# OCR-D/ocrd_keraslm

Hardware: AMD Instinct MI355X
Metric: chars/sec training (stacked-LSTM forward+backward+Adam) (higher is better)
Workload: dtype bf16; 1 GPU; cfg2: depth=2 width=512 length=256 V=256 1 context, stateful training, 3072 streams/GPU, synthetic 10M-char corpus (SURVEY.md 8d); streams_per_gpu=3072, global_batch=3072, seq_len=256, parallelism=dp1

## Files before the change

include/keraslm_hip.h:

```cpp
#ifndef KERASLM_HIP_H
#define KERASLM_HIP_H

#include <stddef.h>
#include <stdint.h>

#ifdef __cplusplus
extern "C" {
#endif

#define KL_ABI_VERSION 1

enum {
  KL_OK = 0,
  KL_ERR_SHAPE = 1,
  KL_ERR_LAUNCH = 2,
  KL_ERR_STATE = 3,
  KL_ERR_WORKSPACE = 4,
  KL_ERR_ARG = 5
};

#define KL_PREC_BF16 1
#define KL_PREC_SPLIT 3

typedef struct kl_config {
// ... 47 lines not shown

int kl_assemble_windows(const int32_t* corpus, size_t n_corpus, const int64_t* plan, int B, int T, int n_ctx, int32_t* idx,
                        int32_t* ctx, int32_t* tgt, void* stream);

int kl_adam_step(kl_handle* h, const float* grads, float* m, float* v, int t, float lr, float b1, float b2,
                 float eps, float clip, void* stream);
int kl_adam_step_scaled(kl_handle* h, const float* grads, float grad_scale, float* m, float* v, int t, float lr,
                        float b1, float b2, float eps, float clip, void* stream);

size_t kl_step_workspace_bytes(const kl_handle* h, int n);
int kl_step_batch(kl_handle* h, int n, const int32_t* idx, const int32_t* ctx, float* pool, const int32_t* slot_in,
                  const int32_t* slot_out, float* probs, void* ws, size_t ws_bytes, void* stream);

void* kl_host_alloc(size_t bytes);
void kl_host_free(void* p);
size_t kl_step_host_workspace_bytes(const kl_handle* h, int n);
int kl_step_batch_host(kl_handle* h, int n, const int32_t* idx, const int32_t* ctx, const int32_t* slot_in,
                       const int32_t* slot_out, const int32_t* target, float* pool, int head_k, float* probs_host,
                       float* heads_host, uint32_t* done_host, uint32_t ticket, void* ws, size_t ws_bytes, void* stream);
size_t kl_walk_workspace_bytes(const kl_handle* h, int n, int total);
size_t kl_walk_stage_bytes(const kl_handle* h, int n, int total);
int kl_walk_batch_host(kl_handle* h, int n, const int32_t* len, const int32_t* idx, const int32_t* target,
                       const int32_t* ctx, const int32_t* slot_in, const int32_t* slot_step, float* pool, int head_k,
                       float* tprob_host, float* heads_host, void* stage_host, uint32_t* done_host, uint32_t ticket,
                       void* ws, size_t ws_bytes, void* stream);
int kl_step_wait(const uint32_t* done_host, uint32_t ticket, double timeout_s);

size_t kl_beam_workspace_bytes(const kl_handle* h, int rows, int fan);
int kl_beam_expand(kl_handle* h, int rows, int fan, float floor, const float* probs, const uint8_t* valid,
                   const float* cum_in, const int32_t* slot_new, int32_t zero_slot, int32_t* idx_next,
                   int32_t* slot_in_next, float* cum_next, int32_t* parent_log, int32_t* idx_log, float* cum_log,
                   int32_t* n_live, void* ws, size_t ws_bytes, void* stream);

size_t kl_sample_workspace_bytes(const kl_handle* h, int rows);
int kl_sample_pick(kl_handle* h, int rows, const float* probs, const uint8_t* valid, float temperature, int top_k,
                   float floor, uint64_t seed, uint32_t step, const float* cum_in, int32_t* idx_next, float* cum_next,
                   float* u_log, void* ws, size_t ws_bytes, void* stream);
int kl_sample_pick_from(kl_handle* h, int rows, uint32_t row0, const float* probs, const uint8_t* valid, float temperature,
                        int top_k, float floor, uint64_t seed, uint32_t step, const float* cum_in, int32_t* idx_next,
                        float* cum_next, float* u_log, void* ws, size_t ws_bytes, void* stream);

int kl_state_dist2(const kl_handle* h, int n, const float* pool, const int32_t* a, const int32_t* b, int k,
                   float* out, void* stream);

int kl_trace_enable(kl_handle* h, int on);
int kl_trace_read(kl_handle* h, int kind, int* n_launches, float* total_ms, int* persistent,
                  double* flops_per_launch);
const char* kl_trace_kernel_name(kl_handle* h, int kind);

int kl_test_gemm_tn(const uint16_t* A, const uint16_t* B, void* C, const float* bias, int M, int N, int K, long lda,
                    long ldb, long ldc, int out_mode, int splits, void* stream);
int kl_test_gemm_an(const uint16_t* A_km, const uint16_t* B, float* C, int M, int N, int K, long lda_km, long ldb,
                    long ldc, int c_transposed, int b_km, void* stream);
size_t kl_test_segment_sums_ws_bytes(int B, int T, int n_ctx, int V, int R);
int kl_test_segment_sums_share(int B, int T);
int kl_test_segment_sums(const uint16_t* dZ, long ld, int B, int T, int cols, const int32_t* idx, const int32_t* ctx, int n_ctx,
                         int V, int R, float* dEK, float* dCtxK, void* ws, void* stream);
int kl_test_thin_gemm(const float* A, long lda, const uint16_t* WT_hi, const uint16_t* WT_lo, long ldw, int M, int N,
                      int K, float* C, long ldc, int split, void* stream);
int kl_test_softmax_ce(float* logits, long ld, int rows, int V, const int32_t* tgt, int B, int T, float inv_count, uint16_t* dlogits,
                       long ld_dl, float* rowstat, float* loss_acc, int last_only, void* stream);
int kl_test_logits_ce_ws(const uint16_t* X, const uint16_t* E, const int32_t* tgt, uint16_t* dlogits, float* rowstat, int B, int T,
                         float inv_count, int last_only, void* stream);
int kl_test_logits_ce_w128(const uint16_t* X, const uint16_t* E, const uint16_t* ET, const int32_t* tgt, uint16_t* dlogits, float* dH,
                           float* rowstat, int B, int T, int V, int Vp, float inv_count, int last_only, void* stream);
int kl_test_dh_ws(const uint16_t* dlogits, const uint16_t* ET, uint16_t* dH, long M, void* stream);
int kl_test_rate_topk(const float* logits, long ld, int rows, int V, const int32_t* tgt, int B, int T, int K,
                      float* tprob, int32_t* alt_id, float* alt_p, int32_t* rank, void* stream);

typedef struct kl_window_view {
  int32_t depth, width, B, T;
  int32_t g_interleaved, c_in_cb, dh_bf16, p_bf16_mask, scan2_rows, reserved[7];
  uint64_t off_H[16], off_C[16], off_Cb[16], off_G[16], off_dZ[16];
} kl_window_view;
int kl_test_window_view(const kl_handle* h, int B, int T, const void* ws, kl_window_view* out);

#ifdef __cplusplus
}
#endif
#endif
```

ocrd_keraslm_amd/csrc/api.hip:

```cpp
#include <hip/hip_runtime.h>
#include <stdio.h>
#include <stdlib.h>
#include <string.h>
#include <time.h>

#include <functional>
#include <utility>

#include <vector>

#include "kl_common.h"
#include "kl_kernels.h"

namespace {

inline size_t align_up(size_t x, size_t a) { return (x + a - 1) / a * a; }
inline int round_up_i(int x, int a) { return (x + a - 1) / a * a; }

struct Carver {
  unsigned char* base;
  size_t off = 0;
  explicit Carver(void* b) : base(reinterpret_cast<unsigned char*>(b)) {}
  template <typename T>
  T* take(size_t count) {
// ... 2022 lines not shown
                   int32_t* parent_log, int32_t* idx_log, float* cum_log, int32_t* n_live, void* ws, size_t ws_bytes,
                   void* stream) {
  if (!h || !probs || !cum_in || !slot_new || !idx_next || !slot_in_next || !cum_next || !parent_log || !idx_log || !cum_log ||
      !n_live)
    return KL_ERR_ARG;
  if (rows < 1 || rows > KL_BEAM_MAX_ROWS || fan < 1 || fan > KL_BEAM_MAX_FAN) return KL_ERR_ARG;
  if (!ws || ws_bytes < kl_beam_ws_bytes(rows, fan)) return KL_ERR_WORKSPACE;
  KlBeamExpand a;
  memset(&a, 0, sizeof(a));
  a.rows = rows; a.fan = fan; a.V = h->cfg.voc_size; a.floor = floor;
  a.probs = probs; a.valid = valid; a.cum_in = cum_in; a.slot_new = slot_new; a.zero_slot = zero_slot;
  a.idx_next = idx_next; a.slot_in_next = slot_in_next; a.cum_next = cum_next;
  a.parent_log = parent_log; a.idx_log = idx_log; a.cum_log = cum_log; a.n_live = n_live;
  return kl_launch_beam_expand(a, ws, (hipStream_t)stream);
}

size_t kl_sample_workspace_bytes(const kl_handle* h, int rows) {
  if (!h || rows < 1 || rows > KL_SAMPLE_MAX_ROWS) return 0;
  return kl_sample_ws_bytes(rows, h->cfg.voc_size);
}

int kl_sample_pick_from(kl_handle* h, int rows, uint32_t row0, const float* probs, const uint8_t* valid, float temperature,
                        int top_k, float floor, uint64_t seed, uint32_t step, const float* cum_in, int32_t* idx_next,
                        float* cum_next, float* u_log, void* ws, size_t ws_bytes, void* stream) {
  if (!h || !probs || !cum_in || !idx_next || !cum_next) return KL_ERR_ARG;
  if (rows < 1 || rows > KL_SAMPLE_MAX_ROWS || top_k < 0 || top_k > KL_SAMPLE_MAX_TOPK) return KL_ERR_ARG;
  if (!(temperature >= 0.f) || temperature == INFINITY || !(floor >= 0.f)) return KL_ERR_ARG;
  if (!ws || ws_bytes < kl_sample_ws_bytes(rows, h->cfg.voc_size)) return KL_ERR_WORKSPACE;
  KlSamplePick a;
  memset(&a, 0, sizeof(a));
  a.rows = rows; a.V = h->cfg.voc_size; a.top_k = top_k; a.temperature = temperature; a.floor = floor;
  a.key0 = (unsigned)(seed & 0xffffffffu); a.key1 = (unsigned)(seed >> 32); a.step = step; a.row0 = row0;
  a.probs = probs; a.valid = valid; a.cum_in = cum_in; a.idx_next = idx_next; a.cum_next = cum_next; a.u_log = u_log;
  return kl_launch_sample_pick(a, ws, (hipStream_t)stream);
}

int kl_sample_pick(kl_handle* h, int rows, const float* probs, const uint8_t* valid, float temperature, int top_k, float floor,
                   uint64_t seed, uint32_t step, const float* cum_in, int32_t* idx_next, float* cum_next, float* u_log, void* ws,
                   size_t ws_bytes, void* stream) {
  return kl_sample_pick_from(h, rows, 0, probs, valid, temperature, top_k, floor, seed, step, cum_in, idx_next, cum_next, u_log,
                             ws, ws_bytes, stream);
}

int kl_test_gemm_tn(const uint16_t* A, const uint16_t* B, void* C, const float* bias, int M, int N, int K, long lda,
                    long ldb, long ldc, int out_mode, int splits, void* stream) {
  return kl_launch_gemm_tn(A, B, C, bias, M, N, K, lda, ldb, ldc, out_mode, splits, 1.f, (hipStream_t)stream);
}

int kl_test_gemm_an(const uint16_t* A_km, const uint16_t* B, float* C, int M, int N, int K, long lda_km, long ldb,
                    long ldc, int c_transposed, int b_km, void* stream) {
  return kl_launch_gemm_an(A_km, B, C, M, N, K, lda_km, ldb, ldc, c_transposed, (hipStream_t)stream, b_km);
}

size_t kl_test_segment_sums_ws_bytes(int B, int T, int n_ctx, int V, int R) {
  if (B < 1 || T < 1 || V < 1 || n_ctx < 0 || (n_ctx > 0 && R < 1)) return 0;
  return kl_segment_sums_ws_bytes(B, T, n_ctx, V, R);
}

int kl_test_segment_sums_share(int B, int T) { return B < 1 || T < 1 ? 0 : kl_segment_sums_share((long)B * T); }

int kl_test_segment_sums(const uint16_t* dZ, long ld, int B, int T, int cols, const int32_t* idx, const int32_t* ctx, int n_ctx,
                         int V, int R, float* dEK, float* dCtxK, void* ws, void* stream) {
  return kl_launch_segment_sums(dZ, ld, B, T, cols, idx, ctx, n_ctx, V, R, dEK, dCtxK, ws, (hipStream_t)stream);
}

int kl_test_thin_gemm(const float* A, long lda, const uint16_t* WT_hi, const uint16_t* WT_lo, long ldw, int M, int N,
                      int K, float* C, long ldc, int split, void* stream) {
  KlOperand op;
  memset(&op, 0, sizeof(op));
  op.A = A; op.lda = lda; op.a_is_f32 = 1; op.WT_hi = WT_hi; op.WT_lo = WT_lo; op.ldw = ldw; op.K = K;
  return kl_launch_thin_gemm(&op, M, N, C, ldc, nullptr, split, (hipStream_t)stream);
}

int kl_test_softmax_ce(float* logits, long ld, int rows, int V, const int32_t* tgt, int B, int T, float inv_count, uint16_t* dlogits,
                       long ld_dl, float* rowstat, float* loss_acc, int last_only, void* stream) {
  return kl_launch_softmax_ce(logits, ld, rows, V, tgt, B, T, inv_count, dlogits, ld_dl, loss_acc, rowstat, 1, (hipStream_t)stream, last_only);
}

int kl_test_logits_ce_ws(const uint16_t* X, const uint16_t* E, const int32_t* tgt, uint16_t* dlogits, float* rowstat, int B, int T,
                         float inv_count, int last_only, void* stream) {
  return kl_launch_logits_ce_ws(X, E, tgt, dlogits, rowstat, B, T, 512, 256, 256, inv_count, last_only, (hipStream_t)stream);
}

int kl_test_logits_ce_w128(const uint16_t* X, const uint16_t* E, const uint16_t* ET, const int32_t* tgt, uint16_t* dlogits, float* dH,
                           float* rowstat, int B, int T, int V, int Vp, float inv_count, int last_only, void* stream) {
  return kl_launch_logits_ce_w128(X, E, ET, tgt, dlogits, dH, rowstat, B, T, 128, V, Vp, inv_count, last_only, (hipStream_t)stream);
}

int kl_test_dh_ws(const uint16_t* dlogits, const uint16_t* ET, uint16_t* dH, long M, void* stream) {
  return kl_launch_dh_ws(dlogits, ET, dH, M, 512, 256, (hipStream_t)stream);
}

int kl_test_rate_topk(const float* logits, long ld, int rows, int V, const int32_t* tgt, int B, int T, int K,
                      float* tprob, int32_t* alt_id, float* alt_p, int32_t* rank, void* stream) {
  return kl_launch_rate_topk(logits, ld, rows, V, tgt, B, T, K, tprob, alt_id, alt_p, rank, (hipStream_t)stream);
}

}

extern "C" int kl_test_fwd_step(const uint16_t* A, long lda, const uint16_t* WT, long ldw, int K, int n_ops,
                                int n_rows, int W, int fused, int iters, float* c_out, uint16_t* h_out,
                                void* stream) {
  KlFwdStep st[4];
  if (fused < 1 || fused > 4 || n_ops < 1 || n_ops > 2) return KL_ERR_ARG;
  for (int f = 0; f < fused; ++f) {
    KlFwdStep& S = st[f];
// ... 265 lines not shown
```

ocrd_keraslm_amd/csrc/gemm.hip:

```cpp
#include <stdlib.h>
#include <string.h>

#include "kl_common.h"
#include "kl_kernels.h"

namespace {

constexpr int BN = 128, BK = 64;
constexpr int NTHREADS = 256;

__device__ __forceinline__ int lds_off(int row, int chunk) {
  return row * 128 + ((chunk ^ ((row >> 1) & 7)) << 4);
}

template <int OUT, int BM>
__global__ __launch_bounds__(NTHREADS) void gemm_tn_kernel(
    const bf16_t* __restrict__ A, const bf16_t* __restrict__ B, void* __restrict__ Cv,
    const float* __restrict__ bias, int M, int N, int K, long lda, long ldb, long ldc,
    int k_per_split, float alpha) {
  constexpr int WM = BM / 64;
  constexpr int WN = 4 / WM;
  constexpr int NT = BN / WN / 16;
  constexpr int ALOADS = BM * 8 / NTHREADS;
  extern __shared__ __attribute__((aligned(16))) unsigned char smem[];
// ... 92 lines not shown
          atomicAdd(reinterpret_cast<float*>(Cv) + (long)row * ldc + col, v);
        }
      }
    }
  }
}

template <int BM>
void launch_bm(int out_mode, dim3 grid, hipStream_t stream, const bf16_t* A, const bf16_t* B, void* C, const float* bias,
               int M, int N, int K, long lda, long ldb, long ldc, int k_per_split, float alpha) {
  const size_t lds = 2 * (BM + BN) * 128;
  switch (out_mode) {
    case 0:
      hipLaunchKernelGGL((gemm_tn_kernel<0, BM>), grid, dim3(NTHREADS), lds, stream, A, B, C, bias, M, N, K, lda, ldb, ldc, k_per_split, alpha);
      break;
    case 1:
      hipLaunchKernelGGL((gemm_tn_kernel<1, BM>), grid, dim3(NTHREADS), lds, stream, A, B, C, bias, M, N, K, lda, ldb, ldc, k_per_split, alpha);
      break;
    default:
      hipLaunchKernelGGL((gemm_tn_kernel<2, BM>), grid, dim3(NTHREADS), lds, stream, A, B, C, bias, M, N, K, lda, ldb, ldc, k_per_split, alpha);
      break;
  }
}


#ifndef KL_GEMM_PRIO
#define KL_GEMM_PRIO 1
#endif
constexpr int LBM = 256, LBN = 128, LSTAGES = 3;

typedef __attribute__((address_space(3))) void lds_void_t;
typedef __attribute__((ext_vector_type(4))) unsigned int u32x4g;

__device__ __forceinline__ void glds16(__amdgpu_buffer_rsrc_t rsrc, unsigned voff, int soff, unsigned lds_addr) {
  unsigned keep;
  asm volatile(
      "s_mov_b32 %0, m0\n\ts_mov_b32 m0, %3\n\ts_nop 0\n\tbuffer_load_dwordx4 %1, %2, %4 offen lds\n\ts_mov_b32 m0, %0"
      : "=&s"(keep)
      : "v"(voff), "s"(rsrc), "s"(lds_addr), "s"(soff)
      : "memory");
}

typedef __attribute__((ext_vector_type(4))) short s16x4;
typedef __attribute__((address_space(3))) s16x4 lds_s16x4;

struct KlGemmSecond {
  const bf16_t* B;
  void* C;
  int n_first, N;
  long ldb, ldc;
  int c_transposed;
};

template <int OUT, bool ILV, int RF, int WM, int WN, bool ATR = false, bool BTR = false>
__global__ __launch_bounds__(64 * WM * WN, 1) void gemm_tn_long_kernel(
    const bf16_t* __restrict__ A, const bf16_t* __restrict__ B_, void* __restrict__ Cv_,
    const float* __restrict__ bias, int M, int N_, int K, long lda, long ldb_, long ldc_,
    int k_per_split, float alpha, const KlGateEpi epi, int xcd_remap, int c_t_, const KlGemmSecond second) {
  const bf16_t* __restrict__ B = B_;
  void* __restrict__ Cv = Cv_;
  int N = N_, c_t = c_t_;
  long ldb = ldb_, ldc = ldc_;
  static_assert(!(ATR || BTR) || (RF == 4 && WM == 4 && WN == 2), "K-major operands: 256 x 128 tiles only");
  constexpr bool PRIO = KL_GEMM_PRIO;
  constexpr int NW = WM * WN;
  constexpr int WROWS = 16 * RF;
  constexpr int TBM = WROWS * WM;
  constexpr int WCOLS = LBN / WN;
  constexpr int NT = WCOLS / 16;
  constexpr int PA = TBM / 8 / NW;
  constexpr int PB = LBN / 8 / NW;
  constexpr int NP = PA + PB;
  constexpr int NP0 = (NP + 1) / 2;
  static_assert(PA >= 1 && PB >= 1 && NP <= 6, "piece split");
  constexpr int STAGE_BYTES = (TBM + LBN) * 128;
  extern __shared__ __attribute__((aligned(16))) unsigned char smem[];
  const int tid = threadIdx.x;
  const int lane = tid & 63;
  const int wave = __builtin_amdgcn_readfirstlane(tid >> 6);
  const int wm = wave / WN, wn = wave % WN;
  int bx = blockIdx.x, by = blockIdx.y, bz = blockIdx.z;
  {
    const unsigned nx = gridDim.x, ny = gridDim.y, total = nx * ny * gridDim.z;
    if (xcd_remap && (total & 7) == 0) {
      const unsigned lin = bx + nx * (by + ny * bz);
      const unsigned re = (lin & 7) * (total >> 3) + (lin >> 3);
      bx = re % nx;
      by = (re / nx) % ny;
      bz = re / (nx * ny);
    }
  }
  const int m0 = by * TBM;
  int n0 = bx * LBN;
  if (second.B != nullptr) {
    if (n0 >= second.n_first) {
      n0 -= second.n_first;
      B = second.B;
      Cv = second.C;
      N = second.N;
      ldb = second.ldb;
      ldc = second.ldc;
      c_t = second.c_transposed;
    } else {
      N = second.n_first;
    }
  }
  const int kbeg = bz * k_per_split;
  const int kend = min(K, kbeg + k_per_split);
  const int nkt = (kend - kbeg) / BK;

  auto clamp31 = [](long v) { return (int)(v > 0x7fffffffL ? 0x7fffffffL : (v < 0 ? 0 : v)); };
  const __amdgpu_buffer_rsrc_t rsA = ATR
      ? __builtin_amdgcn_make_buffer_rsrc(const_cast<bf16_t*>(A + (long)kbeg * lda + m0), 0, clamp31(((long)(kend - kbeg - 1) * lda + (M - m0)) * 2), 0x00020000)
      : __builtin_amdgcn_make_buffer_rsrc(const_cast<bf16_t*>(A + (long)m0 * lda), 0, clamp31(((long)(M - m0 - 1) * lda + K) * 2), 0x00020000);
  const __amdgpu_buffer_rsrc_t rsB = BTR
      ? __builtin_amdgcn_make_buffer_rsrc(const_cast<bf16_t*>(B + (long)kbeg * ldb + n0), 0, clamp31(((long)(kend - kbeg - 1) * ldb + (N - n0)) * 2), 0x00020000)
      : __builtin_amdgcn_make_buffer_rsrc(const_cast<bf16_t*>(B + (long)n0 * ldb), 0, clamp31(((long)(N - n0 - 1) * ldb + K) * 2), 0x00020000);
  unsigned vo[NP];
#pragma unroll
  for (int j = 0; j < NP; ++j) {
    if (ATR && j < PA) {
      const int krow = 2 * (wave * PA + j) + (lane >> 5);
      const int c = (lane & 31) ^ (2 * ((krow & 3) | (((krow >> 3) & 1) << 2)));
      vo[j] = (unsigned)((long)krow * lda * 2 + c * 16);
      continue;
    }
    if (BTR && j >= PA) {
      const int krow = 4 * (wave * PB + (j - PA)) + (lane >> 4);
      const int c = (lane & 15) ^ (2 * ((krow & 3) | (((krow >> 3) & 1) << 2)));
      vo[j] = (unsigned)((long)krow * ldb * 2 + c * 16);
      continue;
    }
    const int row = j < PA ? wave * 8 * PA + j * 8 + (lane >> 3) : wave * 8 * PB + (j - PA) * 8 + (lane >> 3);
    const int c = (lane & 7) ^ ((row >> 1) & 7);
    vo[j] = (unsigned)((long)row * (j < PA ? lda : ldb) * 2 + c * 16);
  }
  const unsigned lds0 = (unsigned)(size_t)(lds_void_t*)smem;
  auto issue_half = [&](int kt, int stage, int half) {
    const int soff = (kbeg + kt * BK) * 2;
    const int soff_a = ATR ? (int)((long)kt * BK * lda * 2) : soff;
    const int soff_b = BTR ? (int)((long)kt * BK * ldb * 2) : soff;
    const unsigned sa = lds0 + stage * STAGE_BYTES + wave * 8 * PA * 128;
    const unsigned sb = lds0 + stage * STAGE_BYTES + TBM * 128 + wave * 8 * PB * 128;
#pragma unroll
    for (int j = half ? NP0 : 0; j < (half ? NP : NP0); ++j) {
      if (j < PA) glds16(rsA, vo[j], soff_a, sa + j * 1024);
      else glds16(rsB, vo[j], soff_b, sb + (j - PA) * 1024);
    }
  };
  auto issue = [&](int kt, int stage) {
    issue_half(kt, stage, 0);
    issue_half(kt, stage, 1);
  };

  f32x4 acc[RF][NT];
#pragma unroll
  for (int i = 0; i < RF; ++i)
#pragma unroll
    for (int j = 0; j < NT; ++j) acc[i][j] = f32x4{0.f, 0.f, 0.f, 0.f};

  if (nkt > 0) issue(0, 0);
  if (nkt > 1) issue(1, 1);
  const int fr = lane & 15, fq = lane >> 4;
  unsigned atr_off[RF];
  if (ATR) {
    const int q = fr >> 2, pp = fr & 3;
    const int fl = 2 * (q | ((fq & 1) << 2));
#pragma unroll
    for (int i = 0; i < RF; ++i)
      atr_off[i] = (unsigned)((fq * 8 + q) * 512 + ((((wm * WROWS + i * 16) >> 3) ^ fl) + (pp >> 1)) * 16 + 8 * (pp & 1));
  }
  unsigned btr_off[NT];
  if (BTR) {
    const int q = fr >> 2, pp = fr & 3;
    const int fl = 2 * (q | ((fq & 1) << 2));
#pragma unroll
    for (int j = 0; j < NT; ++j)
      btr_off[j] = (unsigned)((fq * 8 + q) * 256 + ((((wn * WCOLS + j * 16) >> 3) ^ fl) + (pp >> 1)) * 16 + 8 * (pp & 1));
  }
  int stage = 0;
  for (int kt = 0; kt < nkt; ++kt) {
    if (kt + 1 < nkt) asm volatile("s_waitcnt vmcnt(%0)" ::"n"(NP) : "memory");
    else asm volatile("s_waitcnt vmcnt(0)" ::: "memory");
    __builtin_amdgcn_s_barrier();
    const bool more = kt + 2 < nkt;
    const int nstage = stage >= 1 ? stage - 1 : LSTAGES - 1;
    if (!ILV && more) issue(kt + 2, nstage);
    const unsigned char* a_base = smem + stage * STAGE_BYTES;
    const unsigned char* b_base = a_base + TBM * 128;
#pragma unroll
    for (int s = 0; s < 2; ++s) {
      frag16 fa[RF], fb[NT];
#pragma unroll
      for (int i = 0; i < RF; ++i) {
        if (ATR) {
          const unsigned char* ap = a_base + atr_off[i] + s * 32 * 512;
          const s16x4 lo = __builtin_amdgcn_ds_read_tr16_b64_v4i16((lds_s16x4*)(ap));
          const s16x4 hi = __builtin_amdgcn_ds_read_tr16_b64_v4i16((lds_s16x4*)(ap + 4 * 512));
          fa[i].s[0] = (bf16_t)lo.x; fa[i].s[1] = (bf16_t)lo.y; fa[i].s[2] = (bf16_t)lo.z; fa[i].s[3] = (bf16_t)lo.w;
          fa[i].s[4] = (bf16_t)hi.x; fa[i].s[5] = (bf16_t)hi.y; fa[i].s[6] = (bf16_t)hi.z; fa[i].s[7] = (bf16_t)hi.w;
        } else {
          fa[i].u = *reinterpret_cast<const uint4*>(a_base + lds_off(wm * WROWS + i * 16 + fr, s * 4 + fq));
        }
      }
#pragma unroll
      for (int j = 0; j < NT; ++j) {
        if (BTR) {
          const unsigned char* bp = b_base + btr_off[j] + s * 32 * 256;
          const s16x4 lo = __builtin_amdgcn_ds_read_tr16_b64_v4i16((lds_s16x4*)(bp));
          const s16x4 hi = __builtin_amdgcn_ds_read_tr16_b64_v4i16((lds_s16x4*)(bp + 4 * 256));
          fb[j].s[0] = (bf16_t)lo.x; fb[j].s[1] = (bf16_t)lo.y; fb[j].s[2] = (bf16_t)lo.z; fb[j].s[3] = (bf16_t)lo.w;
          fb[j].s[4] = (bf16_t)hi.x; fb[j].s[5] = (bf16_t)hi.y; fb[j].s[6] = (bf16_t)hi.z; fb[j].s[7] = (bf16_t)hi.w;
        } else {
          fb[j].u = *reinterpret_cast<const uint4*>(b_base + lds_off(wn * WCOLS + j * 16 + fr, s * 4 + fq));
        }
      }
      if (ILV && more) issue_half(kt + 2, nstage, s);
      if (PRIO) __builtin_amdgcn_s_setprio(1);
#pragma unroll
      for (int i = 0; i < RF; ++i)
#pragma unroll
        for (int j = 0; j < NT; ++j) acc[i][j] = mfma16(fa[i].v, fb[j].v, acc[i][j]);
      if (PRIO) __builtin_amdgcn_s_setprio(0);
    }
    stage = stage + 1 < LSTAGES ? stage + 1 : 0;
  }

  if (OUT == 3) {
    constexpr int LDP = LBN + 4;
    float* ct = reinterpret_cast<float*>(smem);
    __builtin_amdgcn_s_barrier();
#pragma unroll
    for (int i = 0; i < RF; ++i)
#pragma unroll
      for (int j = 0; j < NT; ++j)
#pragma unroll
        for (int r = 0; r < 4; ++r)
          ct[(wm * WROWS + i * 16 + fq * 4 + r) * LDP + wn * WCOLS + j * 16 + fr] = acc[i][j][r];
    __syncthreads();
    const int u = tid & 31;
    const int U = bx * 32 + u;
    const int W = epi.W;
    float bg[4] = {0.f, 0.f, 0.f, 0.f};
    if (epi.bias) {
#pragma unroll
      for (int g = 0; g < 4; ++g) bg[g] = epi.bias[(long)g * W + U];
    }
    constexpr int RPP = 64 * NW / 32;
    for (int p = 0; p < TBM / RPP; ++p) {
      const int lrow = p * RPP + (tid >> 5);
      const int row = m0 + lrow;
      if (row >= M) continue;
      float z[4];
#pragma unroll
      for (int g = 0; g < 4; ++g) z[g] = ct[lrow * LDP + g * 32 + u] + bg[g];
      if (epi.T1) {
        const float* t1 = epi.T1 + (long)(epi.i1 ? epi.i1[row] : row) * 4 * W + U;
#pragma unroll
        for (int g = 0; g < 4; ++g) z[g] += t1[(long)g * W];
      }
      if (epi.T2) {
        const float* t2 = epi.T2 + (long)(epi.i2 ? epi.i2[row] : row) * 4 * W + U;
#pragma unroll
        for (int g = 0; g < 4; ++g) z[g] += t2[(long)g * W];
      }
      const float gi = sigmoidf_(z[0]), gf = sigmoidf_(z[1]), gg = tanhf_(z[2]), go = sigmoidf_(z[3]);
      const float cp = epi.c_prev[(long)epi.slot_in[row] * epi.c_ld + U];
      const float c = gf * cp + gi * gg;
      const float hv = go * tanhf_(c);
      const long o = (long)epi.slot_out[row] * epi.out_ld + U;
      epi.c_out[o] = c;
      epi.h_out[o] = hv;
      if (epi.xn) {
        bf16_t hi, lo;
        split_bf16(hv, hi, lo);
        bf16_t* x = epi.xn + (long)row * epi.ldn + U;
        x[0] = hi;
        if (epi.nbn == 3) {
// ... 305 lines not shown
    dim3 grid((N + LBN - 1) / LBN, (M + LBM - 1) / LBM, sp);
    const int e = launch_long(out_mode, grid, stream, A, B, C, bias, M, N, K, lda, ldb, ldc, kps, alpha);
    if (e != 0) return e;
    return hipGetLastError() == hipSuccess ? 0 : KL_ERR_LAUNCH;
  }
  static const bool small_all = getenv("KL_GEMM_SMALL_ALL") && getenv("KL_GEMM_SMALL_ALL")[0] == '1';
  static const bool pers = !(getenv("KL_GEMM_PERS") && getenv("KL_GEMM_PERS")[0] == '0');
  if (pers && !small_all && long_mode >= 2 && long_ok && (out_mode == 0 || out_mode == 1) && K >= 6 * BK && K <= 16 * BK && (N & 3) == 0 && (ldc & 3) == 0 &&
      ((size_t)C & 15) == 0 && (bias == nullptr || N <= 2048) &&
      (long)((M + LBM - 1) / LBM) * ((N + LBN - 1) / LBN) >= 512) {
    static int n_wg = 0;
    if (!n_wg) {
      int dev = 0;
      hipDeviceProp_t prop;
      n_wg = (hipGetDevice(&dev) == hipSuccess && hipGetDeviceProperties(&prop, dev) == hipSuccess && prop.multiProcessorCount >= 8)
                 ? (prop.multiProcessorCount & ~7) : 256;
    }
    const int tiles_n = (N + LBN - 1) / LBN, total = ((M + LBM - 1) / LBM) * tiles_n;
    const size_t lds = (size_t)LSTAGES * (LBM + LBN) * 128 + (bias ? (size_t)N * 4 : 0);
    static KlLdsGrant grant;
    if (kl_grant_lds(grant, reinterpret_cast<const void*>(&gemm_tn_pers_kernel), (size_t)LSTAGES * (LBM + LBN) * 128 + 2048 * 4)) return KL_ERR_LAUNCH;
    hipLaunchKernelGGL(gemm_tn_pers_kernel, dim3(n_wg), dim3(512), lds, stream, A, B, (float*)C, bias, M, N, K, lda, ldb, ldc,
                       alpha, tiles_n, total, out_mode == 1 ? 1 : 0);
    return hipGetLastError() == hipSuccess ? 0 : KL_ERR_LAUNCH;
  }
  if (!small_all && long_mode >= 2 && long_ok && splits == 1 && K >= 256 && (long)((M + LBM - 1) / LBM) * ((N + LBN - 1) / LBN) >= 256) {
    dim3 grid((N + LBN - 1) / LBN, (M + LBM - 1) / LBM, 1);
    const int e = launch_long(out_mode, grid, stream, A, B, C, bias, M, N, K, lda, ldb, ldc, K, alpha);
    if (e != 0) return e;
    return hipGetLastError() == hipSuccess ? 0 : KL_ERR_LAUNCH;
  }
  if (long_mode >= 2 && long_ok && splits == 1 && K >= 512 && M >= 256 &&
      (long)((M + 63) / 64) * ((N + LBN - 1) / LBN) >= 64) {
    dim3 grid((N + LBN - 1) / LBN, (M + 63) / 64, 1);
    const int e = launch_long_t<2, 2, 4>(out_mode, grid, stream, A, B, C, bias, M, N, K, lda, ldb, ldc, K, alpha);
    if (e != 0) return e;
    return hipGetLastError() == hipSuccess ? 0 : KL_ERR_LAUNCH;
  }
  int k_per_split = (K + splits - 1) / splits;
  k_per_split = ((k_per_split + BK - 1) / BK) * BK;
  splits = (K + k_per_split - 1) / k_per_split;
  const int nbx = (N + BN - 1) / BN;
  const bool small = (long)nbx * ((M + 127) / 128) * splits < 256 && M > 64;
  if (small) {
    dim3 grid(nbx, (M + 63) / 64, splits);
    launch_bm<64>(out_mode, grid, stream, A, B, C, bias, M, N, K, lda, ldb, ldc, k_per_split, alpha);
  } else {
    dim3 grid(nbx, (M + 127) / 128, splits);
    launch_bm<128>(out_mode, grid, stream, A, B, C, bias, M, N, K, lda, ldb, ldc, k_per_split, alpha);
  }
  return hipGetLastError() == hipSuccess ? 0 : KL_ERR_LAUNCH;
}

static int an_rows_per_split(int M, int n_all, int K, long ld_max) {
  if (M <= 0 || n_all <= 0 || K <= 0 || (M % LBM) || (K % BK)) return 0;
  const int tiles = (M / LBM) * ((n_all + LBN - 1) / LBN);
  int sp = (256 + tiles - 1) / tiles;
  const int nk = K / BK;
  if (sp > nk / 16) sp = nk / 16;
  if (sp < 1) sp = 1;
  int kps = ((nk + sp - 1) / sp) * BK;
  while ((long)kps * ld_max * 2 >= 0x7fffffffL && kps > BK) {
    ++sp;
    kps = ((nk + sp - 1) / sp) * BK;
  }
  return (long)kps * ld_max * 2 < 0x7fffffffL ? kps : 0;
}

bool kl_gemm_an_applicable(int M, int N, int K, long lda_km) {
  if (lda_km & 7) return false;
  return an_rows_per_split(M, N, K, lda_km) > 0;
}

int kl_launch_gemm_an2(const bf16_t* A_km, const bf16_t* B, float* C, int M, int N, int K, long lda_km, long ldb, long ldc,
                       int c_transposed, const bf16_t* B2, float* C2, int N2, long ldb2, long ldc2, int c_transposed2,
                       hipStream_t stream, int b_km) {
  if (M <= 0 || N <= 0 || K <= 0) return 0;
  if (B2 != nullptr && ((N % LBN) || N2 <= 0 || (ldb2 & 7) || (!b_km && ldb2 >= (1L << 22)))) return KL_ERR_SHAPE;
  const int n_all = B2 != nullptr ? N + N2 : N;
  if ((lda_km & 7) || (ldb & 7) || (!b_km && ldb >= (1L << 22))) return KL_ERR_SHAPE;
  long ld_max = lda_km;
  if (b_km && ldb > ld_max) ld_max = ldb;
  if (b_km && B2 != nullptr && ldb2 > ld_max) ld_max = ldb2;
  const int kps = an_rows_per_split(M, n_all, K, ld_max);
  if (kps <= 0) return KL_ERR_SHAPE;
  const int sp = (K + kps - 1) / kps;
  dim3 grid((n_all + LBN - 1) / LBN, M / LBM, sp);
  KlGateEpi epi;
  memset(&epi, 0, sizeof(epi));
  KlGemmSecond second;
  memset(&second, 0, sizeof(second));
  if (B2 != nullptr) {
    second.B = B2;
    second.C = C2;
    second.n_first = N;
    second.N = N2;
    second.ldb = ldb2;
    second.ldc = ldc2;
    second.c_transposed = c_transposed2;
  }
  const size_t lds = (size_t)LSTAGES * (LBM + LBN) * 128;
  static const int remap = !(getenv("KL_GEMM_XCD") && getenv("KL_GEMM_XCD")[0] == '0');
  static KlLdsGrant grant_a, grant_b;
  if (kl_grant_lds(grant_a, reinterpret_cast<const void*>(&gemm_tn_long_kernel<2, true, 4, 4, 2, true, false>), lds)) return KL_ERR_LAUNCH;
  if (kl_grant_lds(grant_b, reinterpret_cast<const void*>(&gemm_tn_long_kernel<2, true, 4, 4, 2, true, true>), lds)) return KL_ERR_LAUNCH;
  if (b_km)
    hipLaunchKernelGGL((gemm_tn_long_kernel<2, true, 4, 4, 2, true, true>), grid, dim3(512), lds, stream, A_km, B, (void*)C,
                       (const float*)nullptr, M, N, K, lda_km, ldb, ldc, kps, 1.f, epi, remap, c_transposed, second);
  else
    hipLaunchKernelGGL((gemm_tn_long_kernel<2, true, 4, 4, 2, true, false>), grid, dim3(512), lds, stream, A_km, B, (void*)C,
                       (const float*)nullptr, M, N, K, lda_km, ldb, ldc, kps, 1.f, epi, remap, c_transposed, second);
  return hipGetLastError() == hipSuccess ? 0 : KL_ERR_LAUNCH;
}

int kl_launch_gemm_an(const bf16_t* A_km, const bf16_t* B, float* C, int M, int N, int K, long lda_km, long ldb, long ldc,
                      int c_transposed, hipStream_t stream, int b_km) {
  return kl_launch_gemm_an2(A_km, B, C, M, N, K, lda_km, ldb, ldc, c_transposed, nullptr, nullptr, 0, 0, 0, 0, stream, b_km);
}

int kl_launch_gemm_gates(const bf16_t* A3, const bf16_t* WTperm, int n, int W, int Kc, long lda, const KlGateEpi* epi,
                         hipStream_t stream) {
  if (n < 1 || (W & 31) || (Kc % BK) != 0 || (lda & 7) || lda >= (1L << 22) || !epi) return KL_ERR_SHAPE;
  dim3 grid(4 * W / LBN, (n + 63) / 64, 1);
  const int e = launch_long_t<2, 2, 4>(3, grid, stream, A3, WTperm, nullptr, nullptr, n, 4 * W, Kc, lda, lda, 0, Kc, 1.f, epi);
  if (e != 0) return e;
  return hipGetLastError() == hipSuccess ? 0 : KL_ERR_LAUNCH;
}
```

ocrd_keraslm_amd/lib/hipabi.py:

```python
from __future__ import annotations

import ctypes as C
import os

_HERE = os.path.dirname(os.path.abspath(__file__))
LIB_PATH = os.environ.get("KL_LIB") or os.path.join(os.path.dirname(_HERE), "libkeraslm_hip.so")

KL_PREC_BF16 = 1
KL_PREC_SPLIT = 3
KL_RATE_ALTS_MAX = 8
KL_SAMPLE_MAX_ROWS = 1024
KL_SAMPLE_MAX_TOPK = 64


class KlConfig(C.Structure):
    _fields_ = [("depth", C.c_int32), ("width", C.c_int32), ("voc_size", C.c_int32),
                ("n_ctx", C.c_int32), ("ctx_vocab", C.c_int32), ("ctx_dim", C.c_int32)]


class KlWindowView(C.Structure):
    _fields_ = [("depth", C.c_int32), ("width", C.c_int32), ("B", C.c_int32), ("T", C.c_int32),
                ("g_interleaved", C.c_int32), ("c_in_cb", C.c_int32), ("dh_bf16", C.c_int32), ("p_bf16_mask", C.c_int32),
                ("scan2_rows", C.c_int32), ("reserved", C.c_int32 * 7),
                ("off_H", C.c_uint64 * 16), ("off_C", C.c_uint64 * 16), ("off_Cb", C.c_uint64 * 16),
# ... 21 lines not shown
    "kl_rate_workspace_bytes": (C.c_size_t, [C.c_void_p, C.c_int, C.c_int]),
    "kl_rate_window": (C.c_int, [C.c_void_p, C.c_int, C.c_int, C.c_void_p, C.c_void_p, C.c_void_p, C.c_void_p,
                                 C.c_void_p, C.c_void_p, C.c_void_p, C.c_void_p, C.c_size_t, C.c_void_p]),
    "kl_rate_alts_workspace_bytes": (C.c_size_t, [C.c_void_p, C.c_int, C.c_int, C.c_int]),
    "kl_rate_window_alts": (C.c_int, [C.c_void_p, C.c_int, C.c_int, C.c_int, C.c_void_p, C.c_void_p, C.c_void_p, C.c_void_p,
                                      C.c_void_p, C.c_void_p, C.c_void_p, C.c_void_p, C.c_void_p, C.c_void_p, C.c_void_p,
                                      C.c_size_t, C.c_void_p]),
    "kl_train_window": (C.c_int, [C.c_void_p, C.c_int, C.c_int, C.c_void_p, C.c_void_p, C.c_void_p, C.c_void_p,
                                  C.c_void_p, C.c_void_p, C.c_void_p, C.c_void_p, C.c_size_t, C.c_void_p]),
    "kl_assemble_windows": (C.c_int, [C.c_void_p, C.c_size_t, C.c_void_p, C.c_int, C.c_int, C.c_int, C.c_void_p, C.c_void_p,
                                      C.c_void_p, C.c_void_p]),
    "kl_adam_step": (C.c_int, [C.c_void_p, C.c_void_p, C.c_void_p, C.c_void_p, C.c_int, C.c_float, C.c_float,
                               C.c_float, C.c_float, C.c_float, C.c_void_p]),
    "kl_adam_step_scaled": (C.c_int, [C.c_void_p, C.c_void_p, C.c_float, C.c_void_p, C.c_void_p, C.c_int, C.c_float, C.c_float,
                                     C.c_float, C.c_float, C.c_float, C.c_void_p]),
    "kl_step_workspace_bytes": (C.c_size_t, [C.c_void_p, C.c_int]),
    "kl_step_batch": (C.c_int, [C.c_void_p, C.c_int, C.c_void_p, C.c_void_p, C.c_void_p, C.c_void_p, C.c_void_p,
                                C.c_void_p, C.c_void_p, C.c_size_t, C.c_void_p]),
    "kl_host_alloc": (C.c_void_p, [C.c_size_t]),
    "kl_host_free": (None, [C.c_void_p]),
    "kl_step_host_workspace_bytes": (C.c_size_t, [C.c_void_p, C.c_int]),
    "kl_step_batch_host": (C.c_int, [C.c_void_p, C.c_int, C.c_void_p, C.c_void_p, C.c_void_p, C.c_void_p, C.c_void_p,
                                     C.c_void_p, C.c_int, C.c_void_p, C.c_void_p, C.c_void_p, C.c_uint32, C.c_void_p,
                                     C.c_size_t, C.c_void_p]),
    "kl_walk_workspace_bytes": (C.c_size_t, [C.c_void_p, C.c_int, C.c_int]),
    "kl_walk_stage_bytes": (C.c_size_t, [C.c_void_p, C.c_int, C.c_int]),
    "kl_walk_batch_host": (C.c_int, [C.c_void_p, C.c_int, C.c_void_p, C.c_void_p, C.c_void_p, C.c_void_p, C.c_void_p,
                                     C.c_void_p, C.c_void_p, C.c_int, C.c_void_p, C.c_void_p, C.c_void_p, C.c_void_p,
                                     C.c_uint32, C.c_void_p, C.c_size_t, C.c_void_p]),
    "kl_beam_workspace_bytes": (C.c_size_t, [C.c_void_p, C.c_int, C.c_int]),
    "kl_beam_expand": (C.c_int, [C.c_void_p, C.c_int, C.c_int, C.c_float, C.c_void_p, C.c_void_p, C.c_void_p, C.c_void_p,
                                 C.c_int32, C.c_void_p, C.c_void_p, C.c_void_p, C.c_void_p, C.c_void_p, C.c_void_p,
                                 C.c_void_p, C.c_void_p, C.c_size_t, C.c_void_p]),
    "kl_sample_workspace_bytes": (C.c_size_t, [C.c_void_p, C.c_int]),
    "kl_sample_pick": (C.c_int, [C.c_void_p, C.c_int, C.c_void_p, C.c_void_p, C.c_float, C.c_int, C.c_float, C.c_uint64,
                                 C.c_uint32, C.c_void_p, C.c_void_p, C.c_void_p, C.c_void_p, C.c_void_p, C.c_size_t,
                                 C.c_void_p]),
    "kl_sample_pick_from": (C.c_int, [C.c_void_p, C.c_int, C.c_uint32, C.c_void_p, C.c_void_p, C.c_float, C.c_int, C.c_float,
                                      C.c_uint64, C.c_uint32, C.c_void_p, C.c_void_p, C.c_void_p, C.c_void_p, C.c_void_p,
                                      C.c_size_t, C.c_void_p]),
    "kl_step_wait": (C.c_int, [C.c_void_p, C.c_uint32, C.c_double]),
    "kl_state_dist2": (C.c_int, [C.c_void_p, C.c_int, C.c_void_p, C.c_void_p, C.c_void_p, C.c_int, C.c_void_p,
                                 C.c_void_p]),
    "kl_trace_enable": (C.c_int, [C.c_void_p, C.c_int]),
    "kl_set_window_mode": (C.c_int, [C.c_void_p, C.c_int]),
    "kl_set_loss_rows": (C.c_int, [C.c_void_p, C.c_int]),
    "kl_trace_kernel_name": (C.c_char_p, [C.c_void_p, C.c_int]),
    "kl_trace_read": (C.c_int, [C.c_void_p, C.c_int, C.POINTER(C.c_int), C.POINTER(C.c_float), C.POINTER(C.c_int),
                                C.POINTER(C.c_double)]),
    "kl_test_gemm_tn": (C.c_int, [C.c_void_p, C.c_void_p, C.c_void_p, C.c_void_p, C.c_int, C.c_int, C.c_int,
                                  C.c_long, C.c_long, C.c_long, C.c_int, C.c_int, C.c_void_p]),
    "kl_test_gemm_an": (C.c_int, [C.c_void_p, C.c_void_p, C.c_void_p, C.c_int, C.c_int, C.c_int, C.c_long, C.c_long,
                                  C.c_long, C.c_int, C.c_int, C.c_void_p]),
    "kl_test_segment_sums_ws_bytes": (C.c_size_t, [C.c_int, C.c_int, C.c_int, C.c_int, C.c_int]),
    "kl_test_segment_sums_share": (C.c_int, [C.c_int, C.c_int]),
    "kl_test_segment_sums": (C.c_int, [C.c_void_p, C.c_long, C.c_int, C.c_int, C.c_int, C.c_void_p, C.c_void_p, C.c_int,
                                       C.c_int, C.c_int, C.c_void_p, C.c_void_p, C.c_void_p, C.c_void_p]),
    "kl_test_thin_gemm": (C.c_int, [C.c_void_p, C.c_long, C.c_void_p, C.c_void_p, C.c_long, C.c_int, C.c_int,
                                    C.c_int, C.c_void_p, C.c_long, C.c_int, C.c_void_p]),
    "kl_test_softmax_ce": (C.c_int, [C.c_void_p, C.c_long, C.c_int, C.c_int, C.c_void_p, C.c_int, C.c_int, C.c_float,
                                     C.c_void_p, C.c_long, C.c_void_p, C.c_void_p, C.c_int, C.c_void_p]),
    "kl_test_logits_ce_ws": (C.c_int, [C.c_void_p, C.c_void_p, C.c_void_p, C.c_void_p, C.c_void_p, C.c_int, C.c_int,
                                       C.c_float, C.c_int, C.c_void_p]),
    "kl_test_logits_ce_w128": (C.c_int, [C.c_void_p, C.c_void_p, C.c_void_p, C.c_void_p, C.c_void_p, C.c_void_p, C.c_void_p,
                                         C.c_int, C.c_int, C.c_int, C.c_int, C.c_float, C.c_int, C.c_void_p]),
    "kl_test_dh_ws": (C.c_int, [C.c_void_p, C.c_void_p, C.c_void_p, C.c_long, C.c_void_p]),
    "kl_test_rate_topk": (C.c_int, [C.c_void_p, C.c_long, C.c_int, C.c_int, C.c_void_p, C.c_int, C.c_int, C.c_int,
                                    C.c_void_p, C.c_void_p, C.c_void_p, C.c_void_p, C.c_void_p]),
    "kl_test_window_view": (C.c_int, [C.c_void_p, C.c_int, C.c_int, C.c_void_p, C.POINTER(KlWindowView)]),
}

_lib = None


def load():
    global _lib
    if _lib is not None:
        return _lib
    if not os.path.exists(LIB_PATH):
        raise KlError("HIP extension %s not built: run `make -C ocrd_keraslm_amd/csrc` "
                      "(the Rater has no CPU fallback)" % LIB_PATH)
    lib = C.CDLL(LIB_PATH)
    for name, (res, args) in SIGNATURES.items():
        fn = getattr(lib, name)
        fn.restype = res
        fn.argtypes = args
    _lib = lib
    return lib


def check(code, what=""):
    if code != 0:
        msg = load().kl_error_string(code).decode()
        raise KlError("%s failed: %s (code %d)" % (what or "keraslm_hip call", msg, code))
```

Baseline: 34.06 million chars/s.

## Add 256-wide K-major weight-gradient GEMM tiles with deeper ring and fragment prefetch

Adds a wide variant of the long GEMM kernel for the weight-gradient (A^T·B, K-major) path: 256x256 output tiles on sixteen waves, 32-deep K stages, and a 4- or 5-stage LDS ring. In the 5-stage form, LDS fragments for the next step are read while the current MFMAs run. The wider tiles are meant to raise operand reuse per byte loaded and hide LDS and global latency better. The cost is more LDS per block, fewer blocks or splits across the grid, and more register pressure. The path is on by default when N is a multiple of 256, and can be turned off with an environment variable.

Result: faster. 34.71 million chars/s, median of 6 (+1.9%).

```diff
diff --git a/include/keraslm_hip.h b/include/keraslm_hip.h
--- a/include/keraslm_hip.h
+++ b/include/keraslm_hip.h
@@ -123,6 +123,9 @@
                     long ldb, long ldc, int out_mode, int splits, void* stream);
 int kl_test_gemm_an(const uint16_t* A_km, const uint16_t* B, float* C, int M, int N, int K, long lda_km, long ldb,
                     long ldc, int c_transposed, int b_km, void* stream);
+int kl_test_gemm_an2(const uint16_t* A_km, const uint16_t* B, float* C, int M, int N, int K, long lda_km, long ldb, long ldc,
+                     int c_transposed, const uint16_t* B2, float* C2, int N2, long ldb2, long ldc2, int c_transposed2, int b_km,
+                     void* stream);
 size_t kl_test_segment_sums_ws_bytes(int B, int T, int n_ctx, int V, int R);
 int kl_test_segment_sums_share(int B, int T);
 int kl_test_segment_sums(const uint16_t* dZ, long ld, int B, int T, int cols, const int32_t* idx, const int32_t* ctx, int n_ctx,
diff --git a/ocrd_keraslm_amd/csrc/api.hip b/ocrd_keraslm_amd/csrc/api.hip
--- a/ocrd_keraslm_amd/csrc/api.hip
+++ b/ocrd_keraslm_amd/csrc/api.hip
@@ -2098,6 +2098,13 @@
   return kl_launch_gemm_an(A_km, B, C, M, N, K, lda_km, ldb, ldc, c_transposed, (hipStream_t)stream, b_km);
 }
 
+int kl_test_gemm_an2(const uint16_t* A_km, const uint16_t* B, float* C, int M, int N, int K, long lda_km, long ldb, long ldc,
+                     int c_transposed, const uint16_t* B2, float* C2, int N2, long ldb2, long ldc2, int c_transposed2, int b_km,
+                     void* stream) {
+  return kl_launch_gemm_an2(A_km, B, C, M, N, K, lda_km, ldb, ldc, c_transposed, B2, C2, N2, ldb2, ldc2, c_transposed2,
+                            (hipStream_t)stream, b_km);
+}
+
 size_t kl_test_segment_sums_ws_bytes(int B, int T, int n_ctx, int V, int R) {
   if (B < 1 || T < 1 || V < 1 || n_ctx < 0 || (n_ctx > 0 && R < 1)) return 0;
   return kl_segment_sums_ws_bytes(B, T, n_ctx, V, R);
diff --git a/ocrd_keraslm_amd/csrc/gemm.hip b/ocrd_keraslm_amd/csrc/gemm.hip
--- a/ocrd_keraslm_amd/csrc/gemm.hip
+++ b/ocrd_keraslm_amd/csrc/gemm.hip
@@ -168,7 +168,7 @@
   int c_transposed;
 };
 
-template <int OUT, bool ILV, int RF, int WM, int WN, bool ATR = false, bool BTR = false>
+template <int OUT, bool ILV, int RF, int WM, int WN, bool ATR = false, bool BTR = false, int TBN = LBN, int KD = 64, int NST = LSTAGES, bool PFR = false>
 __global__ __launch_bounds__(64 * WM * WN, 1) void gemm_tn_long_kernel(
     const bf16_t* __restrict__ A, const bf16_t* __restrict__ B_, void* __restrict__ Cv_,
     const float* __restrict__ bias, int M, int N_, int K, long lda, long ldb_, long ldc_,
@@ -177,19 +177,24 @@
   void* __restrict__ Cv = Cv_;
   int N = N_, c_t = c_t_;
   long ldb = ldb_, ldc = ldc_;
-  static_assert(!(ATR || BTR) || (RF == 4 && WM == 4 && WN == 2), "K-major operands: 256 x 128 tiles only");
+  static_assert(!(ATR || BTR) || (RF == 4 && WM == 4 && WN == 2 && TBN == 128) || (RF == 4 && WM == 4 && WN == 4 && TBN == 256),
+                "K-major operands: 256 x 128 tiles, or 256 x 256 on sixteen waves");
+  static_assert((TBN == 128 && KD == 64 && NST == 3) || (TBN == 256 && KD == 32 && NST >= 3 && OUT == 2 && ATR && BTR),
+                "256-column tiles: K-major operands, 32-deep stages, split-K atomics");
   constexpr bool PRIO = KL_GEMM_PRIO;
   constexpr int NW = WM * WN;
   constexpr int WROWS = 16 * RF;
   constexpr int TBM = WROWS * WM;
-  constexpr int WCOLS = LBN / WN;
+  constexpr int WCOLS = TBN / WN;
   constexpr int NT = WCOLS / 16;
-  constexpr int PA = TBM / 8 / NW;
-  constexpr int PB = LBN / 8 / NW;
+  constexpr int PA = TBM * KD / 512 / NW;
+  constexpr int PB = TBN * KD / 512 / NW;
   constexpr int NP = PA + PB;
   constexpr int NP0 = (NP + 1) / 2;
   static_assert(PA >= 1 && PB >= 1 && NP <= 6, "piece split");
-  constexpr int STAGE_BYTES = (TBM + LBN) * 128;
+  constexpr int STAGE_BYTES = (TBM + TBN) * KD * 2;
+  constexpr int A_BYTES = TBM * KD * 2;
+  constexpr int BROW = TBN * 2;
   extern __shared__ __attribute__((aligned(16))) unsigned char smem[];
   const int tid = threadIdx.x;
   const int lane = tid & 63;
@@ -207,7 +212,7 @@
     }
   }
   const int m0 = by * TBM;
-  int n0 = bx * LBN;
+  int n0 = bx * TBN;
   if (second.B != nullptr) {
     if (n0 >= second.n_first) {
       n0 -= second.n_first;
@@ -223,7 +228,7 @@
   }
   const int kbeg = bz * k_per_split;
   const int kend = min(K, kbeg + k_per_split);
-  const int nkt = (kend - kbeg) / BK;
+  const int nkt = (kend - kbeg) / KD;
 
   auto clamp31 = [](long v) { return (int)(v > 0x7fffffffL ? 0x7fffffffL : (v < 0 ? 0 : v)); };
   const __amdgpu_buffer_rsrc_t rsA = ATR
@@ -242,8 +247,9 @@
       continue;
     }
     if (BTR && j >= PA) {
-      const int krow = 4 * (wave * PB + (j - PA)) + (lane >> 4);
-      const int c = (lane & 15) ^ (2 * ((krow & 3) | (((krow >> 3) & 1) << 2)));
+      constexpr int LPR = BROW / 16;
+      const int krow = (64 / LPR) * (wave * PB + (j - PA)) + lane / LPR;
+      const int c = (lane & (LPR - 1)) ^ (2 * ((krow & 3) | (((krow >> 3) & 1) << 2)));
       vo[j] = (unsigned)((long)krow * ldb * 2 + c * 16);
       continue;
     }
@@ -253,11 +259,11 @@
   }
   const unsigned lds0 = (unsigned)(size_t)(lds_void_t*)smem;
   auto issue_half = [&](int kt, int stage, int half) {
-    const int soff = (kbeg + kt * BK) * 2;
-    const int soff_a = ATR ? (int)((long)kt * BK * lda * 2) : soff;
-    const int soff_b = BTR ? (int)((long)kt * BK * ldb * 2) : soff;
+    const int soff = (kbeg + kt * KD) * 2;
+    const int soff_a = ATR ? (int)((long)kt * KD * lda * 2) : soff;
+    const int soff_b = BTR ? (int)((long)kt * KD * ldb * 2) : soff;
     const unsigned sa = lds0 + stage * STAGE_BYTES + wave * 8 * PA * 128;
-    const unsigned sb = lds0 + stage * STAGE_BYTES + TBM * 128 + wave * 8 * PB * 128;
+    const unsigned sb = lds0 + stage * STAGE_BYTES + A_BYTES + wave * 8 * PB * 128;
 #pragma unroll
     for (int j = half ? NP0 : 0; j < (half ? NP : NP0); ++j) {
       if (j < PA) glds16(rsA, vo[j], soff_a, sa + j * 1024);
@@ -275,8 +281,12 @@
 #pragma unroll
     for (int j = 0; j < NT; ++j) acc[i][j] = f32x4{0.f, 0.f, 0.f, 0.f};
 
+  constexpr int AHEAD = NST - 1;
   if (nkt > 0) issue(0, 0);
   if (nkt > 1) issue(1, 1);
+  if (AHEAD > 2 && nkt > 2) issue(2, 2);
+  if (AHEAD > 3 && nkt > 3) issue(3, 3);
+  static_assert(AHEAD <= 4, "ring start-up");
   const int fr = lane & 15, fq = lane >> 4;
   unsigned atr_off[RF];
   if (ATR) {
@@ -292,20 +302,62 @@
     const int fl = 2 * (q | ((fq & 1) << 2));
 #pragma unroll
     for (int j = 0; j < NT; ++j)
-      btr_off[j] = (unsigned)((fq * 8 + q) * 256 + ((((wn * WCOLS + j * 16) >> 3) ^ fl) + (pp >> 1)) * 16 + 8 * (pp & 1));
+      btr_off[j] = (unsigned)((fq * 8 + q) * BROW + ((((wn * WCOLS + j * 16) >> 3) ^ fl) + (pp >> 1)) * 16 + 8 * (pp & 1));
   }
   int stage = 0;
-  for (int kt = 0; kt < nkt; ++kt) {
-    if (kt + 1 < nkt) asm volatile("s_waitcnt vmcnt(%0)" ::"n"(NP) : "memory");
+  if (PFR) {
+    static_assert(!PFR || (ATR && BTR && KD == 32 && NST >= 4), "fragment prefetch: the wide form");
+    frag16 fa[RF], fb[NT];
+    auto read_tr = [&](const unsigned char* p, int rowbytes) {
+      frag16 f;
+      const s16x4 lo = __builtin_amdgcn_ds_read_tr16_b64_v4i16((lds_s16x4*)(p));
+      const s16x4 hi = __builtin_amdgcn_ds_read_tr16_b64_v4i16((lds_s16x4*)(p + 4 * rowbytes));
+      const uint2 l = __builtin_bit_cast(uint2, lo), h = __builtin_bit_cast(uint2, hi);
+      f.u = uint4{l.x, l.y, h.x, h.y};
+      return f;
+    };
+    if (nkt > 0) {
+      if (nkt >= AHEAD) asm volatile("s_waitcnt vmcnt(%0)" ::"n"((AHEAD - 1) * NP) : "memory");
+      else asm volatile("s_waitcnt vmcnt(0)" ::: "memory");
+      __builtin_amdgcn_s_barrier();
+#pragma unroll
+      for (int i = 0; i < RF; ++i) fa[i] = read_tr(smem + atr_off[i], 512);
+#pragma unroll
+      for (int j = 0; j < NT; ++j) fb[j] = read_tr(smem + A_BYTES + btr_off[j], BROW);
+    }
+    for (int kt = 0; kt < nkt; ++kt) {
+      if (kt + AHEAD - 1 < nkt) asm volatile("s_waitcnt vmcnt(%0)" ::"n"((AHEAD - 2) * NP) : "memory");
+      else asm volatile("s_waitcnt vmcnt(0)" ::: "memory");
+      __builtin_amdgcn_s_barrier();
+      const int nstage = stage >= 1 ? stage - 1 : NST - 1;
+      if (kt + AHEAD < nkt) issue(kt + AHEAD, nstage);
+      stage = stage + 1 < NST ? stage + 1 : 0;
+      const unsigned char* a_base = smem + stage * STAGE_BYTES;
+      const unsigned char* b_base = a_base + A_BYTES;
+#pragma unroll
+      for (int i = 0; i < RF; ++i) {
+        if (PRIO) __builtin_amdgcn_s_setprio(1);
+#pragma unroll
+        for (int j = 0; j < NT; ++j) acc[i][j] = mfma16(fa[i].v, fb[j].v, acc[i][j]);
+        if (PRIO) __builtin_amdgcn_s_setprio(0);
+        fa[i] = read_tr(a_base + atr_off[i], 512);
+      }
+#pragma unroll
+      for (int j = 0; j < NT; ++j) fb[j] = read_tr(b_base + btr_off[j], BROW);
+    }
+  }
+  for (int kt = PFR ? nkt : 0; kt < nkt; ++kt) {
+    if (kt + AHEAD - 1 < nkt) asm volatile("s_waitcnt vmcnt(%0)" ::"n"((AHEAD - 1) * NP) : "memory");
     else asm volatile("s_waitcnt vmcnt(0)" ::: "memory");
     __builtin_amdgcn_s_barrier();
-    const bool more = kt + 2 < nkt;
-    const int nstage = stage >= 1 ? stage - 1 : LSTAGES - 1;
-    if (!ILV && more) issue(kt + 2, nstage);
+    const bool more = kt + AHEAD < nkt;
+    const int nstage = stage >= 1 ? stage - 1 : NST - 1;
+    if (!ILV && more) issue(kt + AHEAD, nstage);
     const unsigned char* a_base = smem + stage * STAGE_BYTES;
-    const unsigned char* b_base = a_base + TBM * 128;
-#pragma unroll
-    for (int s = 0; s < 2; ++s) {
+    const unsigned char* b_base = a_base + A_BYTES;
+    constexpr int NS = KD / 32;
+#pragma unroll
+    for (int s = 0; s < NS; ++s) {
       frag16 fa[RF], fb[NT];
 #pragma unroll
       for (int i = 0; i < RF; ++i) {
@@ -322,16 +374,19 @@
 #pragma unroll
       for (int j = 0; j < NT; ++j) {
         if (BTR) {
-          const unsigned char* bp = b_base + btr_off[j] + s * 32 * 256;
+          const unsigned char* bp = b_base + btr_off[j] + s * 32 * BROW;
           const s16x4 lo = __builtin_amdgcn_ds_read_tr16_b64_v4i16((lds_s16x4*)(bp));
-          const s16x4 hi = __builtin_amdgcn_ds_read_tr16_b64_v4i16((lds_s16x4*)(bp + 4 * 256));
+          const s16x4 hi = __builtin_amdgcn_ds_read_tr16_b64_v4i16((lds_s16x4*)(bp + 4 * BROW));
           fb[j].s[0] = (bf16_t)lo.x; fb[j].s[1] = (bf16_t)lo.y; fb[j].s[2] = (bf16_t)lo.z; fb[j].s[3] = (bf16_t)lo.w;
           fb[j].s[4] = (bf16_t)hi.x; fb[j].s[5] = (bf16_t)hi.y; fb[j].s[6] = (bf16_t)hi.z; fb[j].s[7] = (bf16_t)hi.w;
         } else {
           fb[j].u = *reinterpret_cast<const uint4*>(b_base + lds_off(wn * WCOLS + j * 16 + fr, s * 4 + fq));
         }
       }
-      if (ILV && more) issue_half(kt + 2, nstage, s);
+      if (ILV && more) {
+        issue_half(kt + AHEAD, nstage, s);
+        if (NS == 1) issue_half(kt + AHEAD, nstage, 1);
+      }
       if (PRIO) __builtin_amdgcn_s_setprio(1);
 #pragma unroll
       for (int i = 0; i < RF; ++i)
@@ -339,7 +394,7 @@
         for (int j = 0; j < NT; ++j) acc[i][j] = mfma16(fa[i].v, fb[j].v, acc[i][j]);
       if (PRIO) __builtin_amdgcn_s_setprio(0);
     }
-    stage = stage + 1 < LSTAGES ? stage + 1 : 0;
+    stage = stage + 1 < NST ? stage + 1 : 0;
   }
 
   if (OUT == 3) {
@@ -751,19 +806,25 @@
   return hipGetLastError() == hipSuccess ? 0 : KL_ERR_LAUNCH;
 }
 
-static int an_rows_per_split(int M, int n_all, int K, long ld_max) {
-  if (M <= 0 || n_all <= 0 || K <= 0 || (M % LBM) || (K % BK)) return 0;
-  const int tiles = (M / LBM) * ((n_all + LBN - 1) / LBN);
+static int an_rows_per_split(int M, int n_all, int K, long ld_max, int tbn = LBN, int kd = BK) {
+  if (M <= 0 || n_all <= 0 || K <= 0 || (M % LBM) || (K % kd)) return 0;
+  const int tiles = (M / LBM) * ((n_all + tbn - 1) / tbn);
   int sp = (256 + tiles - 1) / tiles;
-  const int nk = K / BK;
+  const int nk = K / kd;
   if (sp > nk / 16) sp = nk / 16;
   if (sp < 1) sp = 1;
-  int kps = ((nk + sp - 1) / sp) * BK;
-  while ((long)kps * ld_max * 2 >= 0x7fffffffL && kps > BK) {
+  int kps = ((nk + sp - 1) / sp) * kd;
+  while ((long)kps * ld_max * 2 >= 0x7fffffffL && kps > kd) {
     ++sp;
-    kps = ((nk + sp - 1) / sp) * BK;
+    kps = ((nk + sp - 1) / sp) * kd;
   }
   return (long)kps * ld_max * 2 < 0x7fffffffL ? kps : 0;
+}
+
+constexpr int WBN = 256, WBK = 32;
+static bool an_wide(int M, int N, int N2, int b_km) {
+  static const bool on = !(getenv("KL_GEMM_WIDE") && getenv("KL_GEMM_WIDE")[0] == '0');
+  return on && b_km && M > 0 && (M % LBM) == 0 && N > 0 && (N % WBN) == 0 && (N2 % WBN) == 0;
 }
 
 bool kl_gemm_an_applicable(int M, int N, int K, long lda_km) {
@@ -781,10 +842,14 @@
   long ld_max = lda_km;
   if (b_km && ldb > ld_max) ld_max = ldb;
   if (b_km && B2 != nullptr && ldb2 > ld_max) ld_max = ldb2;
-  const int kps = an_rows_per_split(M, n_all, K, ld_max);
+  const bool wide = an_wide(M, N, B2 != nullptr ? N2 : 0, b_km);
+  int kps = wide ? an_rows_per_split(M, n_all, K, ld_max, WBN, WBK) : 0;
+  const bool go_wide = kps > 0;
+  if (!go_wide) kps = an_rows_per_split(M, n_all, K, ld_max);
   if (kps <= 0) return KL_ERR_SHAPE;
   const int sp = (K + kps - 1) / kps;
-  dim3 grid((n_all + LBN - 1) / LBN, M / LBM, sp);
+  const int tbn = go_wide ? WBN : LBN;
+  dim3 grid((n_all + tbn - 1) / tbn, M / LBM, sp);
   KlGateEpi epi;
   memset(&epi, 0, sizeof(epi));
   KlGemmSecond second;
@@ -798,8 +863,23 @@
     second.ldc = ldc2;
     second.c_transposed = c_transposed2;
   }
+  static const int remap = !(getenv("KL_GEMM_XCD") && getenv("KL_GEMM_XCD")[0] == '0');
+  if (go_wide) {
+    static const bool ring4 = getenv("KL_GEMM_WIDE_RING") && getenv("KL_GEMM_WIDE_RING")[0] == '4';
+    static KlLdsGrant grant_5, grant_4;
+    constexpr size_t stage = (size_t)(LBM + WBN) * WBK * 2;
+    if (!ring4 && kl_grant_lds(grant_5, reinterpret_cast<const void*>(&gemm_tn_long_kernel<2, true, 4, 4, 4, true, true, WBN, WBK, 5, true>), 5 * stage) == 0) {
+      hipLaunchKernelGGL((gemm_tn_long_kernel<2, true, 4, 4, 4, true, true, WBN, WBK, 5, true>), grid, dim3(1024), 5 * stage, stream, A_km, B, (void*)C,
+                         (const float*)nullptr, M, N, K, lda_km, ldb, ldc, kps, 1.f, epi, remap, c_transposed, second);
+    } else {
+      (void)hipGetLastError();
+      if (kl_grant_lds(grant_4, reinterpret_cast<const void*>(&gemm_tn_long_kernel<2, true, 4, 4, 4, true, true, WBN, WBK, 4>), 4 * stage)) return KL_ERR_LAUNCH;
+      hipLaunchKernelGGL((gemm_tn_long_kernel<2, true, 4, 4, 4, true, true, WBN, WBK, 4>), grid, dim3(1024), 4 * stage, stream, A_km, B, (void*)C,
+                         (const float*)nullptr, M, N, K, lda_km, ldb, ldc, kps, 1.f, epi, remap, c_transposed, second);
+    }
+    return hipGetLastError() == hipSuccess ? 0 : KL_ERR_LAUNCH;
+  }
   const size_t lds = (size_t)LSTAGES * (LBM + LBN) * 128;
-  static const int remap = !(getenv("KL_GEMM_XCD") && getenv("KL_GEMM_XCD")[0] == '0');
   static KlLdsGrant grant_a, grant_b;
   if (kl_grant_lds(grant_a, reinterpret_cast<const void*>(&gemm_tn_long_kernel<2, true, 4, 4, 2, true, false>), lds)) return KL_ERR_LAUNCH;
   if (kl_grant_lds(grant_b, reinterpret_cast<const void*>(&gemm_tn_long_kernel<2, true, 4, 4, 2, true, true>), lds)) return KL_ERR_LAUNCH;
diff --git a/ocrd_keraslm_amd/lib/hipabi.py b/ocrd_keraslm_amd/lib/hipabi.py
--- a/ocrd_keraslm_amd/lib/hipabi.py
+++ b/ocrd_keraslm_amd/lib/hipabi.py
@@ -97,6 +97,8 @@
                                   C.c_long, C.c_long, C.c_long, C.c_int, C.c_int, C.c_void_p]),
     "kl_test_gemm_an": (C.c_int, [C.c_void_p, C.c_void_p, C.c_void_p, C.c_int, C.c_int, C.c_int, C.c_long, C.c_long,
                                   C.c_long, C.c_int, C.c_int, C.c_void_p]),
+    "kl_test_gemm_an2": (C.c_int, [C.c_void_p, C.c_void_p, C.c_void_p, C.c_int, C.c_int, C.c_int, C.c_long, C.c_long, C.c_long,
+                                   C.c_int, C.c_void_p, C.c_void_p, C.c_int, C.c_long, C.c_long, C.c_int, C.c_int, C.c_void_p]),
     "kl_test_segment_sums_ws_bytes": (C.c_size_t, [C.c_int, C.c_int, C.c_int, C.c_int, C.c_int]),
     "kl_test_segment_sums_share": (C.c_int, [C.c_int, C.c_int]),
     "kl_test_segment_sums": (C.c_int, [C.c_void_p, C.c_long, C.c_int, C.c_int, C.c_int, C.c_void_p, C.c_void_p, C.c_int,
```
